# stm233/image-compression-for-machine

Measured on AMD Instinct MI355X. Metric: images/sec (256x256) cnn-hyperprior (WACNN) training step, higher is better.
Workload: dtype f32; 1 GPU; cnn (WACNN N=192 M=320) train step, lambda=0.0067 MSE, batch 16/GPU synthetic 256x256, Adam lr 1e-4 + aux Adam, clip 1.0; global_batch=16, parallelism=dp1

## Files before the change

image-compression-for-machine_amd/csrc/wgrad_wino.hip:

```cpp
#include <algorithm>
#include <cmath>
#include <cstdlib>
#include <type_traits>
#include "icm_common.h"

namespace icm {

#define WW_MAXG 32
#define WW_ROW 68
#define WW_SIDE (16 * 8 * WW_ROW)
#define WW_BUF (2 * WW_SIDE)

typedef float f32x2 __attribute__((ext_vector_type(2)));
typedef float f32x2u __attribute__((ext_vector_type(2), aligned(4)));
typedef float f32x4u __attribute__((ext_vector_type(4), aligned(4)));

template <int I, int N, class F>
__device__ __forceinline__ void ww_static_for(F&& f) {
  if constexpr (I < N) {
    f(std::integral_constant<int, I>{});
    ww_static_for<I + 1, N>(f);
  }
}

struct WwPtrs {
  const float* gs;
  const float* gb;
  float* ws;
  float* dbias_ws;
};
struct WwDesc {
  WwPtrs g[WW_MAXG];
  long long gs_bs, gb_bs;
  int N, Ca, Cb, H, W, act_s, act_b;
  int TW, TH;
  FastDiv dTW, dTH;
  int ntiles, nchunks, nsplit, natile, nbtile;
};

template <bool VEC>
__global__ __launch_bounds__(512, 2) void wgrad_wino_kernel(const WwDesc d) {
  extern __shared__ __attribute__((aligned(16))) float smem[];
  const int tid = threadIdx.x, lane = tid & 63;
  const int wave = __builtin_amdgcn_readfirstlane(tid >> 6);
  const WwPtrs G = d.g[blockIdx.y];
  int bid = blockIdx.x;
  const int at = bid % d.natile; bid /= d.natile;
  const int bt = bid % d.nbtile;
  const int split = bid / d.nbtile;
  const int a0 = at * 64, b0 = bt * 64;
  const int niter = (d.nchunks - split + d.nsplit - 1) / d.nsplit;
  const int HW = d.H * d.W;

  const int ch_l = wave * 8 + (lane >> 3), tl = lane & 7;
  const bool aok = a0 + ch_l < d.Ca, bok = b0 + ch_l < d.Cb;
  const int offa = (a0 + ch_l) * HW, offb = (b0 + ch_l) * HW;
  float bsum = 0.0f;

  f32x2 ya[2];
  f32x4 xb[4];
  unsigned vmask = 0;
  unsigned oa_cur = 0, ob_cur = 0;
  auto prep = [&](int it) {
    const int tau = (split + it * d.nsplit) * 8 + tl;
    const uint32_t q = fdiv((uint32_t)tau, d.dTW);
    const int tx = tau - (int)q * d.TW;
    const uint32_t n = fdiv(q, d.dTH);
    const int ty = (int)(q - n * (uint32_t)d.TH);
    const bool tok = tau < d.ntiles;
    const int oy = ty * 2, ox = tx * 2;
    oa_cur = (unsigned)(offa + (int)n * (int)d.gs_bs + oy * d.W + ox);
    unsigned m = 0;
    if constexpr (VEC) {
#pragma unroll
      for (int r = 0; r < 2; ++r) m |= (unsigned)(tok && aok && oy + r < d.H) << r;
#pragma unroll
      for (int r = 0; r < 4; ++r) m |= (unsigned)(tok && bok && (unsigned)(oy - 1 + r) < (unsigned)d.H) << (2 + r);
      const bool left = ox == 0, right = ox == d.W - 2;
      m |= (unsigned)left << 8 | (unsigned)right << 9;
      ob_cur = (unsigned)(offb + (int)n * (int)d.gb_bs + (oy - 1) * d.W + (ox - 1) + (left ? 1 : (right ? -1 : 0)));
    } else {
#pragma unroll
      for (int r = 0; r < 2; ++r)
#pragma unroll
        for (int c = 0; c < 2; ++c) m |= (unsigned)(tok && aok && oy + r < d.H && ox + c < d.W) << (2 * r + c);
#pragma unroll
      for (int r = 0; r < 4; ++r)
#pragma unroll
        for (int c = 0; c < 4; ++c)
          m |= (unsigned)(tok && bok && (unsigned)(oy - 1 + r) < (unsigned)d.H && (unsigned)(ox - 1 + c) < (unsigned)d.W) << (4 + 4 * r + c);
      ob_cur = (unsigned)(offb + (int)n * (int)d.gb_bs + (oy - 1) * d.W + (ox - 1));
    }
    vmask = m;
  };
  auto piece = [&](auto kc) {
    constexpr int k = decltype(kc)::value;
    if constexpr (k < 2) {
      constexpr int r = k;
      if constexpr (VEC) {
        const unsigned off = (vmask >> r & 1u) ? oa_cur + r * d.W : 0u;
        const f32x2u v = *reinterpret_cast<const f32x2u*>(G.gs + off);
        ya[r] = f32x2{v[0], v[1]};
      } else {
#pragma unroll
        for (int c = 0; c < 2; ++c) ya[r][c] = G.gs[(vmask >> (2 * r + c) & 1u) ? oa_cur + r * d.W + c : 0u];
      }
    } else {
      constexpr int r = k - 2;
      if constexpr (VEC) {
        const unsigned off = (vmask >> (2 + r) & 1u) ? ob_cur + r * d.W : 0u;
        const f32x4u v = *reinterpret_cast<const f32x4u*>(G.gb + off);
        xb[r] = f32x4{v[0], v[1], v[2], v[3]};
      } else {
#pragma unroll
        for (int c = 0; c < 4; ++c) xb[r][c] = G.gb[(vmask >> (4 + 4 * r + c) & 1u) ? ob_cur + r * d.W + c : 0u];
      }
    }
  };
  float tY[4][2], uX[16];
  auto rowpass = [&]() {
    {
      float y[4];
#pragma unroll
      for (int r = 0; r < 2; ++r)
#pragma unroll
        for (int c = 0; c < 2; ++c) y[2 * r + c] = (vmask >> (VEC ? r : 2 * r + c) & 1u) ? ya[r][c] : 0.0f;
      bsum += (y[0] + y[1]) + (y[2] + y[3]);
#pragma unroll
      for (int c = 0; c < 2; ++c) {
        tY[0][c] = y[0 * 2 + c];
        tY[1][c] = y[0 * 2 + c] + y[1 * 2 + c];
        tY[2][c] = y[0 * 2 + c] - y[1 * 2 + c];
        tY[3][c] = -y[1 * 2 + c];
      }
    }
    {
      float dd[16];
      if constexpr (VEC) {
        const bool left = vmask >> 8 & 1u, right = vmask >> 9 & 1u;
#pragma unroll
        for (int r = 0; r < 4; ++r) {
          const bool rok = vmask >> (2 + r) & 1u;
          const f32x4 v = xb[r];
          const float e0 = left ? 0.0f : (right ? v[1] : v[0]);
          const float e1 = left ? v[0] : (right ? v[2] : v[1]);
          const float e2 = left ? v[1] : (right ? v[3] : v[2]);
          const float e3 = left ? v[2] : (right ? 0.0f : v[3]);
          dd[r * 4 + 0] = rok ? e0 : 0.0f;
          dd[r * 4 + 1] = rok ? e1 : 0.0f;
          dd[r * 4 + 2] = rok ? e2 : 0.0f;
          dd[r * 4 + 3] = rok ? e3 : 0.0f;
        }
      } else {
#pragma unroll
        for (int r = 0; r < 4; ++r)
#pragma unroll
          for (int c = 0; c < 4; ++c) dd[r * 4 + c] = (vmask >> (4 + 4 * r + c) & 1u) ? xb[r][c] : 0.0f;
      }
#pragma unroll
      for (int j = 0; j < 4; ++j) {
        uX[0 * 4 + j] = dd[0 * 4 + j] - dd[2 * 4 + j];
        uX[1 * 4 + j] = dd[1 * 4 + j] + dd[2 * 4 + j];
        uX[2 * 4 + j] = dd[2 * 4 + j] - dd[1 * 4 + j];
        uX[3 * 4 + j] = dd[1 * 4 + j] - dd[3 * 4 + j];
      }
    }
  };
  auto store_part = [&](auto gc, int buf) {
    constexpr int g = decltype(gc)::value;
    float* da = smem + buf * WW_BUF + tl * WW_ROW + ch_l;
    if constexpr (g < 4) {
      constexpr int i = g;
      da[(i * 4 + 0) * 8 * WW_ROW] = tY[i][0];
      da[(i * 4 + 1) * 8 * WW_ROW] = tY[i][0] + tY[i][1];
      da[(i * 4 + 2) * 8 * WW_ROW] = tY[i][0] - tY[i][1];
      da[(i * 4 + 3) * 8 * WW_ROW] = -tY[i][1];
    } else {
      constexpr int i = g - 4;
      float* db = da + WW_SIDE;
      db[(i * 4 + 0) * 8 * WW_ROW] = uX[i * 4 + 0] - uX[i * 4 + 2];
      db[(i * 4 + 1) * 8 * WW_ROW] = uX[i * 4 + 1] + uX[i * 4 + 2];
      db[(i * 4 + 2) * 8 * WW_ROW] = uX[i * 4 + 2] - uX[i * 4 + 1];
      db[(i * 4 + 3) * 8 * WW_ROW] = uX[i * 4 + 1] - uX[i * 4 + 3];
    }
  };

  const int h = lane >> 5, l31 = lane & 31;
  f32x16 acc[2][2][2];
#pragma unroll
  for (int x = 0; x < 2; ++x)
#pragma unroll
    for (int i = 0; i < 2; ++i)
#pragma unroll
      for (int j = 0; j < 2; ++j)
#pragma unroll
        for (int e = 0; e < 16; ++e) acc[x][i][j][e] = 0.0f;
  const int foff = (2 * wave) * 8 * WW_ROW + h * WW_ROW + l31;
  auto multiply = [&](int rd, int wr) {
    const float* pa = smem + rd * WW_BUF + foff;
    const float* pb = pa + WW_SIDE;
    float a0v = pa[0], a1v = pa[32], b0v = pb[0], b1v = pb[32];
    ww_static_for<0, 8>([&](auto gc) {
      constexpr int g = decltype(gc)::value, x = g >> 2;
      float na0 = 0.0f, na1 = 0.0f, nb0 = 0.0f, nb1 = 0.0f;
      if constexpr (g < 7) {
        constexpr int o = (((g + 1) >> 2) * 8 + 2 * ((g + 1) & 3)) * WW_ROW;
        na0 = pa[o]; na1 = pa[o + 32]; nb0 = pb[o]; nb1 = pb[o + 32];
      }
      if constexpr (g < 3) {
        piece(std::integral_constant<int, 2 * g>{});
        piece(std::integral_constant<int, 2 * g + 1>{});
      }
      store_part(gc, wr);
      __builtin_amdgcn_sched_barrier(0);
      acc[x][0][0] = __builtin_amdgcn_mfma_f32_32x32x2f32(a0v, b0v, acc[x][0][0], 0, 0, 0);
      acc[x][0][1] = __builtin_amdgcn_mfma_f32_32x32x2f32(a0v, b1v, acc[x][0][1], 0, 0, 0);
      acc[x][1][0] = __builtin_amdgcn_mfma_f32_32x32x2f32(a1v, b0v, acc[x][1][0], 0, 0, 0);
      acc[x][1][1] = __builtin_amdgcn_mfma_f32_32x32x2f32(a1v, b1v, acc[x][1][1], 0, 0, 0);
      __builtin_amdgcn_sched_barrier(0);
      a0v = na0; a1v = na1; b0v = nb0; b1v = nb1;
    });
  };

  prep(0);
  ww_static_for<0, 6>(piece);
  rowpass();
  ww_static_for<0, 8>([&](auto gc) { store_part(gc, 0); });
  prep(1);
  ww_static_for<0, 6>(piece);
  __syncthreads();
  for (int it = 0; it < niter; ++it) {
    rowpass();
    prep(it + 2);
    multiply(it & 1, (it + 1) & 1);
    __syncthreads();
  }

  if (G.dbias_ws != nullptr && bt == 0) {
    float s = bsum;
    s += __shfl_xor(s, 1, 64);
    s += __shfl_xor(s, 2, 64);
    s += __shfl_xor(s, 4, 64);
    if (tl == 0 && aok) G.dbias_ws[(long long)split * d.Ca + a0 + ch_l] = s;
  }
#pragma unroll
  for (int x = 0; x < 2; ++x) {
    const int xi = 2 * wave + x;
#pragma unroll
    for (int i = 0; i < 2; ++i)
#pragma unroll
      for (int j = 0; j < 2; ++j) {
        const int b = b0 + j * 32 + l31;
        float* row0 = G.ws + (((long long)split * 16 + xi) * d.Ca + a0 + i * 32 + 4 * h) * d.Cb + b;
#pragma unroll
        for (int e = 0; e < 16; ++e) {
          const int ar = (e & 3) + 8 * (e >> 2);
          if (a0 + i * 32 + 4 * h + ar < d.Ca && b < d.Cb) row0[(long long)ar * d.Cb] = acc[x][i][j][e];
        }
        __builtin_amdgcn_sched_barrier(0);
      }
  }
}

int wgrad_wino_plan(const icm_wgrad_args& a, int nproblems, int* nsplit_out, int* nchunks_out) {
  if (a.KH != 3 || a.KW != 3 || a.stride != 1 || a.pad != 1 || a.OH != a.H || a.OW != a.W) return ICM_ERR_UNSUPPORTED;
  if (a.act_s != ICM_ACT_NONE || a.act_b != ICM_ACT_NONE) return ICM_ERR_UNSUPPORTED;
  const int TW = cdiv(a.W, 2), TH = cdiv(a.H, 2);
  const long long ntiles = (long long)a.N * TW * TH;
  if (ntiles >= 65536) return ICM_ERR_UNSUPPORTED;
  if ((long long)a.N * a.gs_bs + (long long)(a.Ca + 64) * a.H * a.W >= (1LL << 30) ||
      (long long)a.N * a.gb_bs + (long long)(a.Cb + 64) * a.H * a.W >= (1LL << 30))
    return ICM_ERR_UNSUPPORTED;
  const int nchunks = (int)((ntiles + 7) / 8);
  const int base = cdiv(a.Ca, 64) * cdiv(a.Cb, 64) * std::max(1, nproblems);
  double best = 1e300;
  int nsplit = 1;
  for (int sp = 1; sp <= std::min(nchunks, 256); ++sp) {
    const double rounds = std::ceil((double)base * sp / 256.0);
    const double per = (double)cdiv(nchunks, sp) + 2.0;
    const double cost = rounds * per * (1.0 + 0.004 * sp);
    if (cost < best - 1e-9) { best = cost; nsplit = sp; }
  }
  *nsplit_out = nsplit;
  *nchunks_out = nchunks;
  return ICM_OK;
}

int launch_wgrad_wino(const icm_wgrad_args* arr, int n, int nsplit, int nchunks, float* const* ws, float* const* dbias_ws,
                      hipStream_t stream) {
  const icm_wgrad_args& a = arr[0];
  WwDesc d{};
  for (int i = 0; i < WW_MAXG; ++i) {
    const int k = i < n ? i : 0;
    d.g[i].gs = arr[k].gs; d.g[i].gb = arr[k].gb; d.g[i].ws = ws[k]; d.g[i].dbias_ws = dbias_ws[k];
  }
  d.gs_bs = a.gs_bs; d.gb_bs = a.gb_bs;
  d.N = a.N; d.Ca = a.Ca; d.Cb = a.Cb; d.H = a.H; d.W = a.W; d.act_s = a.act_s; d.act_b = a.act_b;
  d.TW = cdiv(a.W, 2); d.TH = cdiv(a.H, 2);
  d.dTW = make_fastdiv((uint32_t)d.TW); d.dTH = make_fastdiv((uint32_t)d.TH);
  d.ntiles = a.N * d.TW * d.TH; d.nchunks = nchunks; d.nsplit = nsplit;
  d.natile = cdiv(a.Ca, 64); d.nbtile = cdiv(a.Cb, 64);
  const long long nblk = (long long)d.natile * d.nbtile * nsplit;
  if (nblk <= 0 || nblk > 0x7fffffffLL) return ICM_ERR_ARG;
  const size_t lds = (size_t)2 * WW_BUF * sizeof(float);
  static const bool novec = env_int("ICM_WW_NOVEC", 0) != 0;
  auto fn = (!novec && a.W % 2 == 0 && a.W >= 4) ? wgrad_wino_kernel<true> : wgrad_wino_kernel<false>;
  if (!ensure_max_lds(reinterpret_cast<const void*>(fn))) return ICM_ERR_LAUNCH;
  hipLaunchKernelGGL(fn, dim3((unsigned)nblk, n), dim3(512), lds, stream, d);
  ICM_CHECK_LAUNCH();
  return ICM_OK;
}

}
```

Baseline: 408.9 images/s.

## Interleave Winograd wgrad loads and transforms between MFMAs and skip empty half-tiles

Restructures the Winograd weight-gradient kernel main loop to software-pipeline more finely. Global loads, row transforms and LDS stores are now spread into slots between individual MFMA instructions, with two register sets alternating so loads run one iteration further ahead. It also adds template specializations that skip the MFMAs and stores for the 32-wide half-tiles lying entirely beyond the channel count, for channel counts that are not multiples of 64. The cost is higher register pressure from the doubled load buffers and four times as many kernel instantiations.

New measurement: 407.5 images/s. No clear change (-0.4%).

```diff
diff --git a/image-compression-for-machine_amd/csrc/wgrad_wino.hip b/image-compression-for-machine_amd/csrc/wgrad_wino.hip
--- a/image-compression-for-machine_amd/csrc/wgrad_wino.hip
+++ b/image-compression-for-machine_amd/csrc/wgrad_wino.hip
@@ -38,16 +38,11 @@
   int ntiles, nchunks, nsplit, natile, nbtile;
 };
 
-template <bool VEC>
-__global__ __launch_bounds__(512, 2) void wgrad_wino_kernel(const WwDesc d) {
-  extern __shared__ __attribute__((aligned(16))) float smem[];
+template <bool VEC, bool A2, bool B2>
+__device__ __forceinline__ void ww_block(const WwDesc& d, float* smem, const int at, const int bt, const int split) {
   const int tid = threadIdx.x, lane = tid & 63;
   const int wave = __builtin_amdgcn_readfirstlane(tid >> 6);
   const WwPtrs G = d.g[blockIdx.y];
-  int bid = blockIdx.x;
-  const int at = bid % d.natile; bid /= d.natile;
-  const int bt = bid % d.nbtile;
-  const int split = bid / d.nbtile;
   const int a0 = at * 64, b0 = bt * 64;
   const int niter = (d.nchunks - split + d.nsplit - 1) / d.nsplit;
   const int HW = d.H * d.W;
@@ -57,184 +52,244 @@
   const int offa = (a0 + ch_l) * HW, offb = (b0 + ch_l) * HW;
   float bsum = 0.0f;
 
-  f32x2 ya[2];
-  f32x4 xb[4];
-  unsigned vmask = 0;
-  unsigned oa_cur = 0, ob_cur = 0;
-  auto prep = [&](int it) {
-    const int tau = (split + it * d.nsplit) * 8 + tl;
-    const uint32_t q = fdiv((uint32_t)tau, d.dTW);
-    const int tx = tau - (int)q * d.TW;
-    const uint32_t n = fdiv(q, d.dTH);
-    const int ty = (int)(q - n * (uint32_t)d.TH);
-    const bool tok = tau < d.ntiles;
-    const int oy = ty * 2, ox = tx * 2;
-    oa_cur = (unsigned)(offa + (int)n * (int)d.gs_bs + oy * d.W + ox);
-    unsigned m = 0;
-    if constexpr (VEC) {
-#pragma unroll
-      for (int r = 0; r < 2; ++r) m |= (unsigned)(tok && aok && oy + r < d.H) << r;
-#pragma unroll
-      for (int r = 0; r < 4; ++r) m |= (unsigned)(tok && bok && (unsigned)(oy - 1 + r) < (unsigned)d.H) << (2 + r);
-      const bool left = ox == 0, right = ox == d.W - 2;
-      m |= (unsigned)left << 8 | (unsigned)right << 9;
-      ob_cur = (unsigned)(offb + (int)n * (int)d.gb_bs + (oy - 1) * d.W + (ox - 1) + (left ? 1 : (right ? -1 : 0)));
-    } else {
-#pragma unroll
-      for (int r = 0; r < 2; ++r)
-#pragma unroll
-        for (int c = 0; c < 2; ++c) m |= (unsigned)(tok && aok && oy + r < d.H && ox + c < d.W) << (2 * r + c);
-#pragma unroll
-      for (int r = 0; r < 4; ++r)
-#pragma unroll
-        for (int c = 0; c < 4; ++c)
-          m |= (unsigned)(tok && bok && (unsigned)(oy - 1 + r) < (unsigned)d.H && (unsigned)(ox - 1 + c) < (unsigned)d.W) << (4 + 4 * r + c);
-      ob_cur = (unsigned)(offb + (int)n * (int)d.gb_bs + (oy - 1) * d.W + (ox - 1));
-    }
-    vmask = m;
-  };
-  auto piece = [&](auto kc) {
-    constexpr int k = decltype(kc)::value;
-    if constexpr (k < 2) {
-      constexpr int r = k;
+  const int h = lane >> 5, l31 = lane & 31;
+  f32x16 acc[2][2][2];
+#pragma unroll
+  for (int x = 0; x < 2; ++x)
+#pragma unroll
+    for (int i = 0; i < 2; ++i)
+#pragma unroll
+      for (int j = 0; j < 2; ++j)
+#pragma unroll
+        for (int e = 0; e < 16; ++e) acc[x][i][j][e] = 0.0f;
+  const int foff = (2 * wave) * 8 * WW_ROW + h * WW_ROW + l31;
+
+  auto run = [&](auto la, auto lb) {
+    constexpr bool LA = decltype(la)::value, LB = decltype(lb)::value;
+    f32x2 ya[2][2];
+    f32x4 xb[2][4];
+    unsigned vmask[2] = {0, 0};
+    unsigned oa_cur = 0, ob_cur = 0;
+    auto prep = [&](auto sc, int it) {
+      constexpr int S = decltype(sc)::value;
+      const int tau = (split + it * d.nsplit) * 8 + tl;
+      const uint32_t q = fdiv((uint32_t)tau, d.dTW);
+      const int tx = tau - (int)q * d.TW;
+      const uint32_t n = fdiv(q, d.dTH);
+      const int ty = (int)(q - n * (uint32_t)d.TH);
+      const bool tok = tau < d.ntiles;
+      const int oy = ty * 2, ox = tx * 2;
+      oa_cur = (unsigned)(offa + (int)n * (int)d.gs_bs + oy * d.W + ox);
+      unsigned m = 0;
       if constexpr (VEC) {
-        const unsigned off = (vmask >> r & 1u) ? oa_cur + r * d.W : 0u;
-        const f32x2u v = *reinterpret_cast<const f32x2u*>(G.gs + off);
-        ya[r] = f32x2{v[0], v[1]};
+#pragma unroll
+        for (int r = 0; r < 2; ++r) m |= (unsigned)(tok && aok && oy + r < d.H) << r;
+#pragma unroll
+        for (int r = 0; r < 4; ++r) m |= (unsigned)(tok && bok && (unsigned)(oy - 1 + r) < (unsigned)d.H) << (2 + r);
+        const bool left = ox == 0, right = ox == d.W - 2;
+        m |= (unsigned)left << 8 | (unsigned)right << 9;
+        ob_cur = (unsigned)(offb + (int)n * (int)d.gb_bs + (oy - 1) * d.W + (ox - 1) + (left ? 1 : (right ? -1 : 0)));
       } else {
 #pragma unroll
-        for (int c = 0; c < 2; ++c) ya[r][c] = G.gs[(vmask >> (2 * r + c) & 1u) ? oa_cur + r * d.W + c : 0u];
-      }
-    } else {
-      constexpr int r = k - 2;
-      if constexpr (VEC) {
-        const unsigned off = (vmask >> (2 + r) & 1u) ? ob_cur + r * d.W : 0u;
-        const f32x4u v = *reinterpret_cast<const f32x4u*>(G.gb + off);
-        xb[r] = f32x4{v[0], v[1], v[2], v[3]};
+        for (int r = 0; r < 2; ++r)
+#pragma unroll
+          for (int c = 0; c < 2; ++c) m |= (unsigned)(tok && aok && oy + r < d.H && ox + c < d.W) << (2 * r + c);
+#pragma unroll
+        for (int r = 0; r < 4; ++r)
+#pragma unroll
+          for (int c = 0; c < 4; ++c)
+            m |= (unsigned)(tok && bok && (unsigned)(oy - 1 + r) < (unsigned)d.H && (unsigned)(ox - 1 + c) < (unsigned)d.W) << (4 + 4 * r + c);
+        ob_cur = (unsigned)(offb + (int)n * (int)d.gb_bs + (oy - 1) * d.W + (ox - 1));
+      }
+      vmask[S] = m;
+    };
+    auto piece = [&](auto sc, auto kc) {
+      constexpr int S = decltype(sc)::value, k = decltype(kc)::value;
+      const unsigned vm = vmask[S];
+      if constexpr (k < 2 ? !LA : !LB) {
+      } else if constexpr (k < 2) {
+        constexpr int r = k;
+        if constexpr (VEC) {
+          const unsigned off = (vm >> r & 1u) ? oa_cur + r * d.W : 0u;
+          const f32x2u v = *reinterpret_cast<const f32x2u*>(G.gs + off);
+          ya[S][r] = f32x2{v[0], v[1]};
+        } else {
+#pragma unroll
+          for (int c = 0; c < 2; ++c) ya[S][r][c] = G.gs[(vm >> (2 * r + c) & 1u) ? oa_cur + r * d.W + c : 0u];
+        }
       } else {
-#pragma unroll
-        for (int c = 0; c < 4; ++c) xb[r][c] = G.gb[(vmask >> (4 + 4 * r + c) & 1u) ? ob_cur + r * d.W + c : 0u];
+        constexpr int r = k - 2;
+        if constexpr (VEC) {
+          const unsigned off = (vm >> (2 + r) & 1u) ? ob_cur + r * d.W : 0u;
+          const f32x4u v = *reinterpret_cast<const f32x4u*>(G.gb + off);
+          xb[S][r] = f32x4{v[0], v[1], v[2], v[3]};
+        } else {
+#pragma unroll
+          for (int c = 0; c < 4; ++c) xb[S][r][c] = G.gb[(vm >> (4 + 4 * r + c) & 1u) ? ob_cur + r * d.W + c : 0u];
+        }
+      }
+    };
+    float tY[4][2], uX[16];
+    auto rowpass_a = [&](auto sc) {
+      constexpr int S = decltype(sc)::value;
+      const unsigned vm = vmask[S];
+      if constexpr (LA) {
+        float y[4];
+#pragma unroll
+        for (int r = 0; r < 2; ++r)
+#pragma unroll
+          for (int c = 0; c < 2; ++c) y[2 * r + c] = (vm >> (VEC ? r : 2 * r + c) & 1u) ? ya[S][r][c] : 0.0f;
+        bsum += (y[0] + y[1]) + (y[2] + y[3]);
+#pragma unroll
+        for (int c = 0; c < 2; ++c) {
+          tY[0][c] = y[0 * 2 + c];
+          tY[1][c] = y[0 * 2 + c] + y[1 * 2 + c];
+          tY[2][c] = y[0 * 2 + c] - y[1 * 2 + c];
+          tY[3][c] = -y[1 * 2 + c];
+        }
+      }
+    };
+    float dd1[4], dd2[4];
+    auto rowpass_b = [&](auto sc, auto pc) {
+      constexpr int S = decltype(sc)::value, part = decltype(pc)::value;
+      if constexpr (LB) {
+        const unsigned vm = vmask[S];
+        auto xrow = [&](auto rc, float* o) {
+          constexpr int r = decltype(rc)::value;
+          if constexpr (VEC) {
+            const bool left = vm >> 8 & 1u, right = vm >> 9 & 1u;
+            const bool rok = vm >> (2 + r) & 1u;
+            const f32x4 v = xb[S][r];
+            const float e0 = left ? 0.0f : (right ? v[1] : v[0]);
+            const float e1 = left ? v[0] : (right ? v[2] : v[1]);
+            const float e2 = left ? v[1] : (right ? v[3] : v[2]);
+            const float e3 = left ? v[2] : (right ? 0.0f : v[3]);
+            o[0] = rok ? e0 : 0.0f;
+            o[1] = rok ? e1 : 0.0f;
+            o[2] = rok ? e2 : 0.0f;
+            o[3] = rok ? e3 : 0.0f;
+          } else {
+#pragma unroll
+            for (int c = 0; c < 4; ++c) o[c] = (vm >> (4 + 4 * r + c) & 1u) ? xb[S][r][c] : 0.0f;
+          }
+        };
+        if constexpr (part == 0) {
+          xrow(std::integral_constant<int, 1>{}, dd1);
+          xrow(std::integral_constant<int, 2>{}, dd2);
+#pragma unroll
+          for (int j = 0; j < 4; ++j) {
+            uX[1 * 4 + j] = dd1[j] + dd2[j];
+            uX[2 * 4 + j] = dd2[j] - dd1[j];
+          }
+        } else if constexpr (part == 1) {
+          float dd0[4];
+          xrow(std::integral_constant<int, 0>{}, dd0);
+#pragma unroll
+          for (int j = 0; j < 4; ++j) uX[0 * 4 + j] = dd0[j] - dd2[j];
+        } else {
+          float dd3[4];
+          xrow(std::integral_constant<int, 3>{}, dd3);
+#pragma unroll
+          for (int j = 0; j < 4; ++j) uX[3 * 4 + j] = dd1[j] - dd3[j];
+        }
+      }
+    };
+    auto rowpass = [&](auto sc) {
+      rowpass_a(sc);
+      ww_static_for<0, 3>([&](auto pc) { rowpass_b(sc, pc); });
+    };
+    auto store_part = [&](auto gc, int buf) {
+      constexpr int g = decltype(gc)::value;
+      float* da = smem + buf * WW_BUF + tl * WW_ROW + ch_l;
+      if constexpr (g < 4 ? !LA : !LB) {
+      } else if constexpr (g < 4) {
+        constexpr int i = g;
+        da[(i * 4 + 0) * 8 * WW_ROW] = tY[i][0];
+        da[(i * 4 + 1) * 8 * WW_ROW] = tY[i][0] + tY[i][1];
+        da[(i * 4 + 2) * 8 * WW_ROW] = tY[i][0] - tY[i][1];
+        da[(i * 4 + 3) * 8 * WW_ROW] = -tY[i][1];
+      } else {
+        constexpr int i = g - 4;
+        float* db = da + WW_SIDE;
+        db[(i * 4 + 0) * 8 * WW_ROW] = uX[i * 4 + 0] - uX[i * 4 + 2];
+        db[(i * 4 + 1) * 8 * WW_ROW] = uX[i * 4 + 1] + uX[i * 4 + 2];
+        db[(i * 4 + 2) * 8 * WW_ROW] = uX[i * 4 + 2] - uX[i * 4 + 1];
+        db[(i * 4 + 3) * 8 * WW_ROW] = uX[i * 4 + 1] - uX[i * 4 + 3];
+      }
+    };
+
+    auto multiply = [&](auto pc, int it) {
+      constexpr int P = decltype(pc)::value;
+      using SetG = std::integral_constant<int, P>;
+      using SetT = std::integral_constant<int, 1 - P>;
+      auto slot = [&](auto slc) {
+        constexpr int sl = decltype(slc)::value;
+        auto st = [&](auto gc) { store_part(gc, 1 - P); };
+        if constexpr (sl == 1) rowpass_a(SetT{});
+        if constexpr (sl == 2) rowpass_b(SetT{}, std::integral_constant<int, 0>{});
+        if constexpr (sl == 4) rowpass_b(SetT{}, std::integral_constant<int, 1>{});
+        if constexpr (sl == 6) rowpass_b(SetT{}, std::integral_constant<int, 2>{});
+        if constexpr (sl >= 3 && sl <= 13 && (sl & 1)) piece(SetG{}, std::integral_constant<int, (sl - 3) / 2>{});
+        if constexpr (sl == 3) st(std::integral_constant<int, 0>{});
+        if constexpr (sl == 5) st(std::integral_constant<int, 1>{});
+        if constexpr (sl == 7) st(std::integral_constant<int, 2>{});
+        if constexpr (sl == 8) st(std::integral_constant<int, 5>{});
+        if constexpr (sl == 9) st(std::integral_constant<int, 3>{});
+        if constexpr (sl == 10) st(std::integral_constant<int, 6>{});
+        if constexpr (sl == 11) st(std::integral_constant<int, 4>{});
+        if constexpr (sl == 12) st(std::integral_constant<int, 7>{});
+        if constexpr (sl == 16) prep(SetT{}, it + 3);
+        __builtin_amdgcn_sched_barrier(0);
+      };
+      const float* pa = smem + P * WW_BUF + foff;
+      const float* pb = pa + WW_SIDE;
+      float a0v = pa[0], a1v = A2 ? pa[32] : 0.0f, b0v = pb[0], b1v = B2 ? pb[32] : 0.0f;
+      ww_static_for<0, 8>([&](auto gc) {
+        constexpr int g = decltype(gc)::value, x = g >> 2;
+        float na0 = 0.0f, na1 = 0.0f, nb0 = 0.0f, nb1 = 0.0f;
+        if constexpr (g < 7) {
+          constexpr int o = (((g + 1) >> 2) * 8 + 2 * ((g + 1) & 3)) * WW_ROW;
+          na0 = pa[o]; nb0 = pb[o];
+          if constexpr (A2) na1 = pa[o + 32];
+          if constexpr (B2) nb1 = pb[o + 32];
+        }
+        slot(std::integral_constant<int, 4 * g + 0>{});
+        acc[x][0][0] = __builtin_amdgcn_mfma_f32_32x32x2f32(a0v, b0v, acc[x][0][0], 0, 0, 0);
+        __builtin_amdgcn_sched_barrier(0);
+        slot(std::integral_constant<int, 4 * g + 1>{});
+        if constexpr (B2) acc[x][0][1] = __builtin_amdgcn_mfma_f32_32x32x2f32(a0v, b1v, acc[x][0][1], 0, 0, 0);
+        __builtin_amdgcn_sched_barrier(0);
+        slot(std::integral_constant<int, 4 * g + 2>{});
+        if constexpr (A2) acc[x][1][0] = __builtin_amdgcn_mfma_f32_32x32x2f32(a1v, b0v, acc[x][1][0], 0, 0, 0);
+        __builtin_amdgcn_sched_barrier(0);
+        slot(std::integral_constant<int, 4 * g + 3>{});
+        if constexpr (A2 && B2) acc[x][1][1] = __builtin_amdgcn_mfma_f32_32x32x2f32(a1v, b1v, acc[x][1][1], 0, 0, 0);
+        __builtin_amdgcn_sched_barrier(0);
+        a0v = na0; a1v = na1; b0v = nb0; b1v = nb1;
+      });
+    };
+
+    constexpr std::integral_constant<int, 0> s0{};
+    constexpr std::integral_constant<int, 1> s1{};
+    prep(s0, 0);
+    ww_static_for<0, 6>([&](auto kc) { piece(s0, kc); });
+    rowpass(s0);
+    ww_static_for<0, 8>([&](auto gc) { store_part(gc, 0); });
+    prep(s1, 1);
+    ww_static_for<0, 6>([&](auto kc) { piece(s1, kc); });
+    prep(s0, 2);
+    __syncthreads();
+    for (int it = 0; it < niter; it += 2) {
+      multiply(s0, it);
+      __syncthreads();
+      if (it + 1 < niter) {
+        multiply(s1, it + 1);
+        __syncthreads();
       }
     }
   };
-  float tY[4][2], uX[16];
-  auto rowpass = [&]() {
-    {
-      float y[4];
-#pragma unroll
-      for (int r = 0; r < 2; ++r)
-#pragma unroll
-        for (int c = 0; c < 2; ++c) y[2 * r + c] = (vmask >> (VEC ? r : 2 * r + c) & 1u) ? ya[r][c] : 0.0f;
-      bsum += (y[0] + y[1]) + (y[2] + y[3]);
-#pragma unroll
-      for (int c = 0; c < 2; ++c) {
-        tY[0][c] = y[0 * 2 + c];
-        tY[1][c] = y[0 * 2 + c] + y[1 * 2 + c];
-        tY[2][c] = y[0 * 2 + c] - y[1 * 2 + c];
-        tY[3][c] = -y[1 * 2 + c];
-      }
-    }
-    {
-      float dd[16];
-      if constexpr (VEC) {
-        const bool left = vmask >> 8 & 1u, right = vmask >> 9 & 1u;
-#pragma unroll
-        for (int r = 0; r < 4; ++r) {
-          const bool rok = vmask >> (2 + r) & 1u;
-          const f32x4 v = xb[r];
-          const float e0 = left ? 0.0f : (right ? v[1] : v[0]);
-          const float e1 = left ? v[0] : (right ? v[2] : v[1]);
-          const float e2 = left ? v[1] : (right ? v[3] : v[2]);
-          const float e3 = left ? v[2] : (right ? 0.0f : v[3]);
-          dd[r * 4 + 0] = rok ? e0 : 0.0f;
-          dd[r * 4 + 1] = rok ? e1 : 0.0f;
-          dd[r * 4 + 2] = rok ? e2 : 0.0f;
-          dd[r * 4 + 3] = rok ? e3 : 0.0f;
-        }
-      } else {
-#pragma unroll
-        for (int r = 0; r < 4; ++r)
-#pragma unroll
-          for (int c = 0; c < 4; ++c) dd[r * 4 + c] = (vmask >> (4 + 4 * r + c) & 1u) ? xb[r][c] : 0.0f;
-      }
-#pragma unroll
-      for (int j = 0; j < 4; ++j) {
-        uX[0 * 4 + j] = dd[0 * 4 + j] - dd[2 * 4 + j];
-        uX[1 * 4 + j] = dd[1 * 4 + j] + dd[2 * 4 + j];
-        uX[2 * 4 + j] = dd[2 * 4 + j] - dd[1 * 4 + j];
-        uX[3 * 4 + j] = dd[1 * 4 + j] - dd[3 * 4 + j];
-      }
-    }
-  };
-  auto store_part = [&](auto gc, int buf) {
-    constexpr int g = decltype(gc)::value;
-    float* da = smem + buf * WW_BUF + tl * WW_ROW + ch_l;
-    if constexpr (g < 4) {
-      constexpr int i = g;
-      da[(i * 4 + 0) * 8 * WW_ROW] = tY[i][0];
-      da[(i * 4 + 1) * 8 * WW_ROW] = tY[i][0] + tY[i][1];
-      da[(i * 4 + 2) * 8 * WW_ROW] = tY[i][0] - tY[i][1];
-      da[(i * 4 + 3) * 8 * WW_ROW] = -tY[i][1];
-    } else {
-      constexpr int i = g - 4;
-      float* db = da + WW_SIDE;
-      db[(i * 4 + 0) * 8 * WW_ROW] = uX[i * 4 + 0] - uX[i * 4 + 2];
-      db[(i * 4 + 1) * 8 * WW_ROW] = uX[i * 4 + 1] + uX[i * 4 + 2];
-      db[(i * 4 + 2) * 8 * WW_ROW] = uX[i * 4 + 2] - uX[i * 4 + 1];
-      db[(i * 4 + 3) * 8 * WW_ROW] = uX[i * 4 + 1] - uX[i * 4 + 3];
-    }
-  };
-
-  const int h = lane >> 5, l31 = lane & 31;
-  f32x16 acc[2][2][2];
-#pragma unroll
-  for (int x = 0; x < 2; ++x)
-#pragma unroll
-    for (int i = 0; i < 2; ++i)
-#pragma unroll
-      for (int j = 0; j < 2; ++j)
-#pragma unroll
-        for (int e = 0; e < 16; ++e) acc[x][i][j][e] = 0.0f;
-  const int foff = (2 * wave) * 8 * WW_ROW + h * WW_ROW + l31;
-  auto multiply = [&](int rd, int wr) {
-    const float* pa = smem + rd * WW_BUF + foff;
-    const float* pb = pa + WW_SIDE;
-    float a0v = pa[0], a1v = pa[32], b0v = pb[0], b1v = pb[32];
-    ww_static_for<0, 8>([&](auto gc) {
-      constexpr int g = decltype(gc)::value, x = g >> 2;
-      float na0 = 0.0f, na1 = 0.0f, nb0 = 0.0f, nb1 = 0.0f;
-      if constexpr (g < 7) {
-        constexpr int o = (((g + 1) >> 2) * 8 + 2 * ((g + 1) & 3)) * WW_ROW;
-        na0 = pa[o]; na1 = pa[o + 32]; nb0 = pb[o]; nb1 = pb[o + 32];
-      }
-      if constexpr (g < 3) {
-        piece(std::integral_constant<int, 2 * g>{});
-        piece(std::integral_constant<int, 2 * g + 1>{});
-      }
-      store_part(gc, wr);
-      __builtin_amdgcn_sched_barrier(0);
-      acc[x][0][0] = __builtin_amdgcn_mfma_f32_32x32x2f32(a0v, b0v, acc[x][0][0], 0, 0, 0);
-      acc[x][0][1] = __builtin_amdgcn_mfma_f32_32x32x2f32(a0v, b1v, acc[x][0][1], 0, 0, 0);
-      acc[x][1][0] = __builtin_amdgcn_mfma_f32_32x32x2f32(a1v, b0v, acc[x][1][0], 0, 0, 0);
-      acc[x][1][1] = __builtin_amdgcn_mfma_f32_32x32x2f32(a1v, b1v, acc[x][1][1], 0, 0, 0);
-      __builtin_amdgcn_sched_barrier(0);
-      a0v = na0; a1v = na1; b0v = nb0; b1v = nb1;
-    });
-  };
-
-  prep(0);
-  ww_static_for<0, 6>(piece);
-  rowpass();
-  ww_static_for<0, 8>([&](auto gc) { store_part(gc, 0); });
-  prep(1);
-  ww_static_for<0, 6>(piece);
-  __syncthreads();
-  for (int it = 0; it < niter; ++it) {
-    rowpass();
-    prep(it + 2);
-    multiply(it & 1, (it + 1) & 1);
-    __syncthreads();
-  }
+  if ((A2 && B2) || wave < 4) run(std::true_type{}, std::true_type{});
+  else run(std::bool_constant<A2>{}, std::bool_constant<B2>{});
 
   if (G.dbias_ws != nullptr && bt == 0) {
     float s = bsum;
@@ -250,6 +305,7 @@
     for (int i = 0; i < 2; ++i)
 #pragma unroll
       for (int j = 0; j < 2; ++j) {
+        if ((i == 1 && !A2) || (j == 1 && !B2)) continue;
         const int b = b0 + j * 32 + l31;
         float* row0 = G.ws + (((long long)split * 16 + xi) * d.Ca + a0 + i * 32 + 4 * h) * d.Cb + b;
 #pragma unroll
@@ -260,6 +316,20 @@
         __builtin_amdgcn_sched_barrier(0);
       }
   }
+}
+
+template <bool VEC>
+__global__ __launch_bounds__(512, 2) void wgrad_wino_kernel(const WwDesc d) {
+  extern __shared__ __attribute__((aligned(16))) float smem[];
+  int bid = blockIdx.x;
+  const int at = bid % d.natile; bid /= d.natile;
+  const int bt = bid % d.nbtile;
+  const int split = bid / d.nbtile;
+  const bool a2 = at * 64 + 32 < d.Ca, b2 = bt * 64 + 32 < d.Cb;
+  if (a2 && b2) ww_block<VEC, true, true>(d, smem, at, bt, split);
+  else if (a2) ww_block<VEC, true, false>(d, smem, at, bt, split);
+  else if (b2) ww_block<VEC, false, true>(d, smem, at, bt, split);
+  else ww_block<VEC, false, false>(d, smem, at, bt, split);
 }
 
 int wgrad_wino_plan(const icm_wgrad_args& a, int nproblems, int* nsplit_out, int* nchunks_out) {
```
